# nannau/DoWnGAN

Hardware: AMD Instinct MI355X
Metric: train-step samples/sec (G+D+GP) (higher is better)
Workload: dtype bf16

## Files before the change

downgan_amd/csrc/wgrad.hip:

```cpp
#include "dg_internal.h"

#include <stdlib.h>

struct WGArgs {
  const void* x; const void* u; float* dw;
  long long ldx, ldu;
  int H, W, Ho, Wo, stride, Cin, Cout;
  int u_ps, cps_chunks;
  int Mpix, ppb;
  int nci_t;
  float* db;
  int tri;
  float* dwk[8]; float* dbk[8];
  float* det_ws; const float* det_base; long long det_stride, det_db_off;
  const unsigned char* ex; const unsigned char* eu;
  int grp, ngrp, nunits, gtiles;
};

static void wg_group_order(WGArgs& a, int nco_t, int ntiles, int splits) {
  a.grp = 0;
  if (a.tri || ntiles <= 72) return;
  const int per_co = 3 * a.nci_t;
  int cg = 0;
  for (int c = 1; c <= nco_t; ++c)
    if (nco_t % c == 0 && c * per_co <= 64) cg = c;
  if (!cg) return;
  const double dy_b = (double)a.Mpix * a.Cout, x_b = (double)a.Mpix * a.stride * a.stride * a.Cin;
  const double in_order = 8.0 * dy_b + x_b * (a.nci_t >= 8 ? 1.0 : 8.0 / a.nci_t), grouped = dy_b + x_b * (nco_t / cg);
  if (grouped > 0.8 * in_order) return;
  a.grp = cg * per_co; a.ngrp = nco_t / cg; a.nunits = splits * a.ngrp; a.gtiles = ntiles;
}
static unsigned wg_group_blocks(const WGArgs& a) { return 8u * (unsigned)((a.nunits + 7) / 8) * (unsigned)a.grp; }

__device__ __forceinline__ bool wg_decode(const WGArgs& a, int& bx, int& by) {
  const unsigned lin0 = blockIdx.y * gridDim.x + blockIdx.x;
  if (a.grp) {
    const unsigned xcd = lin0 & 7u, slot = lin0 >> 3;
    const unsigned unit = (slot / (unsigned)a.grp) * 8u + xcd, within = slot % (unsigned)a.grp;
    if (unit >= (unsigned)a.nunits) return false;
    by = (int)(unit / (unsigned)a.ngrp); bx = (int)((unit % (unsigned)a.ngrp) * (unsigned)a.grp + within);
    return true;
  }
  const unsigned lin = gridDim.x <= 72 ? xcd_remap(lin0, gridDim.x * gridDim.y) : lin0;
  bx = (int)(lin % gridDim.x); by = (int)(lin / gridDim.x);
  return true;
}
#define WG_DET_PTR(a, p, by) ((a).det_ws ? (a).det_ws + (long long)(by) * (a).det_stride + ((p) - (a).det_base) : (p))
#define WG_DET_DB(a, by) ((a).det_ws ? (a).det_ws + (long long)(by) * (a).det_stride + (a).det_db_off : (a).db)

typedef __attribute__((address_space(3))) s16x4_t* lds_s16x4_ptr;

typedef __attribute__((ext_vector_type(4))) unsigned int u32x4w_t;
#define WG_OOB_OFF 0x80000000u

template <typename T, int BCO, int BCI, bool ROWSTEP, int KP, bool IM2COL = false>
__global__ __launch_bounds__(256) void wg_kernel(const WGArgs a) {
  constexpr int EPC = DT<T>::EPC;
  constexpr int CPRU = BCO / EPC, CPRX = BCI / EPC;
  constexpr int NU = KP * CPRU / 256, NX = KP * CPRX / 256;
  static_assert(NU >= 1 && NX >= 1, "tile too small");
  constexpr int FA = BCO / 64, FB = BCI / 64;
  constexpr int PADE = sizeof(T) == 2 ? 32 : 0;
  constexpr int LDU = BCO + PADE, LDX = BCI + PADE;
  extern __shared__ __attribute__((aligned(16))) unsigned char wg_dsm[];
  T* const smem = reinterpret_cast<T*>(wg_dsm);

  const int tid = threadIdx.x, lane = tid & 63, wave = tid >> 6;
  const unsigned lin0 = blockIdx.y * gridDim.x + blockIdx.x;
  const unsigned lin = gridDim.x <= 72 ? xcd_remap(lin0, gridDim.x * gridDim.y) : lin0;
  const int bx = (int)(lin % gridDim.x), by = (int)(lin / gridDim.x);
  const int ci_t = IM2COL ? 0 : bx % a.nci_t;
  const int tap = IM2COL ? 4 : (bx / a.nci_t) % 9;
  const int co_t = IM2COL ? bx : bx / (a.nci_t * 9);
  const int co0 = co_t * BCO, ci0 = ci_t * BCI;
  const int dr = tap / 3 - 1, dc = tap % 3 - 1;
  const int pbeg = by * a.ppb;
  const int pend = min(a.Mpix, pbeg + a.ppb);
  const T* __restrict__ X = reinterpret_cast<const T*>(a.x);
  const T* __restrict__ U = reinterpret_cast<const T*>(a.u);

  uint4 ru[NU], rx[NX];
  int s_n = 0, s_ho = 0, s_wo = 0;
  unsigned uoffc[NU], xoffc[NX];
  int xrow[NX];
  constexpr int TPC = EPC / 2;
  unsigned imoff[IM2COL ? NX : 1][TPC];
  if constexpr (ROWSTEP) {
    s_wo = pbeg % a.Wo; const int t = pbeg / a.Wo; s_ho = t % a.Ho; s_n = t / a.Ho;
#pragma unroll
    for (int i = 0; i < NU; ++i) {
      const int e = tid + 256 * i, row = e / CPRU, col = e % CPRU;
      const int co = co0 + col * EPC;
      if (co >= a.Cout) { uoffc[i] = WG_OOB_OFF; continue; }
      if (!a.u_ps) uoffc[i] = (unsigned)(((long long)row * a.ldu + co) * (int)sizeof(T));
      else {
        const int cchunk = co / EPC, q = cchunk / a.cps_chunks, c = cchunk - q * a.cps_chunks;
        uoffc[i] = (unsigned)((((long long)(q >> 1) * (2 * a.Wo) + 2 * row + (q & 1)) * a.ldu + c * EPC) * (int)sizeof(T));
      }
    }
#pragma unroll
    for (int i = 0; i < NX; ++i) {
      const int e = tid + 256 * i, row = e / CPRX, col = e % CPRX;
      const int ci = ci0 + col * EPC;
      xrow[i] = row;
      xoffc[i] = ci < a.Cin ? (unsigned)(((long long)row * a.stride * a.ldx + ci) * (int)sizeof(T)) : WG_OOB_OFF;
      if constexpr (IM2COL) {
#pragma unroll
        for (int tt = 0; tt < TPC; ++tt) {
          const int tp = col * TPC + tt;
          imoff[i][tt] = tp < 9 ? (unsigned)((((long long)(tp / 3) * a.W + row + tp % 3) * a.ldx) * (int)sizeof(T)) : WG_OOB_OFF;
        }
      }
    }
  }
  auto gload_row = [&]() {
    const long long ub = !a.u_ps ? ((long long)(s_n * a.Ho + s_ho) * a.Wo + s_wo) * a.ldu
                                 : ((long long)(s_n * 2 * a.Ho + 2 * s_ho) * (2 * a.Wo) + 2 * s_wo) * a.ldu;
    const int hi = s_ho * a.stride + dr;
    const bool row_ok = (unsigned)hi < (unsigned)a.H;
    const int wi0 = s_wo * a.stride + dc;
    const long long xb = ((long long)(s_n * a.H + hi) * a.W + wi0) * a.ldx;
    __amdgpu_buffer_rsrc_t rU = __builtin_amdgcn_make_buffer_rsrc((void*)(U + ub), 0, (int)WG_OOB_OFF, 0x00020000);
    __amdgpu_buffer_rsrc_t rX = __builtin_amdgcn_make_buffer_rsrc((void*)(X + xb), 0, (int)WG_OOB_OFF, 0x00020000);
#pragma unroll
    for (int i = 0; i < NU; ++i) ru[i] = __builtin_bit_cast(uint4, __builtin_amdgcn_raw_buffer_load_b128(rU, uoffc[i], 0, 0));
    if constexpr (IM2COL) {
      const long long xb2 = ((long long)(s_n * a.H + s_ho - 1) * a.W + s_wo - 1) * a.ldx;
      __amdgpu_buffer_rsrc_t rI = __builtin_amdgcn_make_buffer_rsrc((void*)(X + xb2), 0, (int)WG_OOB_OFF, 0x00020000);
#pragma unroll
      for (int i = 0; i < NX; ++i) {
        const int col = (tid + 256 * i) % CPRX;
        unsigned w[4] = {0u, 0u, 0u, 0u};
#pragma unroll
        for (int tt = 0; tt < TPC; ++tt) {
          const int tp = col * TPC + tt;
          const int hh = s_ho - 1 + tp / 3, ww = s_wo - 1 + xrow[i] + tp % 3;
          const unsigned vo = (tp < 9 && (unsigned)hh < (unsigned)a.H && (unsigned)ww < (unsigned)a.W) ? imoff[i][tt] : WG_OOB_OFF;
          if constexpr (sizeof(T) == 2) {
            unsigned v = __builtin_amdgcn_raw_buffer_load_b32(rI, vo, 0, 0);
            if (tp == 9) v = 0x3f80u;
            w[tt] = v;
          } else {
            typedef __attribute__((ext_vector_type(2))) unsigned int u32x2w_t;
            u32x2w_t v = __builtin_amdgcn_raw_buffer_load_b64(rI, vo, 0, 0);
            if (tp == 9) { v[0] = 0x3f800000u; v[1] = 0u; }
            w[2 * tt] = v[0]; w[2 * tt + 1] = v[1];
          }
        }
        rx[i] = make_uint4(w[0], w[1], w[2], w[3]);
      }
    } else {
#pragma unroll
      for (int i = 0; i < NX; ++i) {
        const int wi = wi0 + xrow[i] * a.stride;
        const unsigned vo = (row_ok && (unsigned)wi < (unsigned)a.W) ? xoffc[i] : WG_OOB_OFF;
// ... 335 lines not shown
    const int hi = s_ho + dr;
    const bool row_ok = (unsigned)hi < (unsigned)a.H;
    const int wi0 = s_wo - 1;
    const long long xb = ((long long)(s_n * a.H + (row_ok ? hi : 0)) * a.W + wi0) * a.ldx;
    __amdgpu_buffer_rsrc_t rU = __builtin_amdgcn_make_buffer_rsrc((void*)(U + ub), 0, (int)WG_OOB_OFF, 0x00020000);
    __amdgpu_buffer_rsrc_t rX = __builtin_amdgcn_make_buffer_rsrc((void*)(X + xb), 0, (int)WG_OOB_OFF, 0x00020000);
#pragma unroll
    for (int i = 0; i < NU; ++i) ru[i] = __builtin_bit_cast(uint4, __builtin_amdgcn_raw_buffer_load_b128(rU, uoffc[i], 0, 0));
#pragma unroll
    for (int i = 0; i < NX; ++i) {
      const int wi = wi0 + xrow[i];
      const unsigned vo = (row_ok && (unsigned)wi < (unsigned)a.W) ? xoffc[i] : WG_OOB_OFF;
      rx[i] = __builtin_bit_cast(uint4, __builtin_amdgcn_raw_buffer_load_b128(rX, vo, 0, 0));
    }
    s_wo += KP;
    if (s_wo >= a.Wo) { s_wo = 0; if (++s_ho == a.Ho) { s_ho = 0; ++s_n; } }
  };
  auto lstore = [&](int buf) {
    T* su = smem + buf * BUF;
    T* sx = su + KP * LDU;
#pragma unroll
    for (int i = 0; i < NU; ++i) {
      const int e = tid + 256 * i, row = e / CPRU, col = e % CPRU;
      if (row < KP) *reinterpret_cast<uint4*>(su + row * LDU + col * EPC) = ru[i];
    }
#pragma unroll
    for (int i = 0; i < NX; ++i) {
      const int e = tid + 256 * i, row = e / CPRX, col = e % CPRX;
      if (row < XR) *reinterpret_cast<uint4*>(sx + row * LDX + col * EPC) = rx[i];
    }
  };

  f32x16_t acc[3][FA][FB];
#pragma unroll
  for (int s = 0; s < 3; ++s)
#pragma unroll
    for (int i = 0; i < FA; ++i)
#pragma unroll
      for (int j = 0; j < FB; ++j)
#pragma unroll
        for (int e = 0; e < 16; ++e) acc[s][i][j][e] = 0.f;

  const int wci = wave;
  const int r32 = lane & 31, h = lane >> 5;
  const int nsteps = (pend - pbeg + KP - 1) / KP;
  if (nsteps <= 0) return;

  gload();
  lstore(0);
  __syncthreads();
  int cur = 0;
  for (int ks = 0; ks < nsteps; ++ks) {
    const bool more = ks + 1 < nsteps;
    if (more) gload();
    const T* su = smem + cur * BUF;
    const T* sx = su + KP * LDU;
    if constexpr (sizeof(T) == 2) {
      const int grp16 = (lane >> 4) & 1, i16 = lane & 15, q = i16 >> 2, pp = i16 & 3;
      typedef __attribute__((ext_vector_type(8))) short s16x8_t;
#pragma unroll
      for (int kk = 0; kk < KP / 16; ++kk) {
        bf16x8_t fa[FA];
        const int k0 = kk * 16 + 8 * h + q;
#pragma unroll
        for (int f = 0; f < FA; ++f) {
          const int ch = 32 * f + 16 * grp16 + 4 * pp;
          s16x4_t lo = __builtin_amdgcn_ds_read_tr16_b64_v4i16((lds_s16x4_ptr)(su + k0 * LDU + ch));
          s16x4_t hi = __builtin_amdgcn_ds_read_tr16_b64_v4i16((lds_s16x4_ptr)(su + (k0 + 4) * LDU + ch));
          s16x8_t v = {lo[0], lo[1], lo[2], lo[3], hi[0], hi[1], hi[2], hi[3]};
          fa[f] = __builtin_bit_cast(bf16x8_t, v);
        }
#pragma unroll
        for (int s = 0; s < 3; ++s) {
          bf16x8_t fb[FB];
#pragma unroll
          for (int f = 0; f < FB; ++f) {
            const int ch = wci * (BCI / 4) + 32 * f + 16 * grp16 + 4 * pp;
            s16x4_t lo = __builtin_amdgcn_ds_read_tr16_b64_v4i16((lds_s16x4_ptr)(sx + (k0 + s) * LDX + ch));
            s16x4_t hi = __builtin_amdgcn_ds_read_tr16_b64_v4i16((lds_s16x4_ptr)(sx + (k0 + s + 4) * LDX + ch));
            s16x8_t v = {lo[0], lo[1], lo[2], lo[3], hi[0], hi[1], hi[2], hi[3]};
            fb[f] = __builtin_bit_cast(bf16x8_t, v);
          }
#pragma unroll
          for (int i = 0; i < FA; ++i)
#pragma unroll
            for (int j = 0; j < FB; ++j)
              acc[s][i][j] = __builtin_amdgcn_mfma_f32_32x32x16_bf16(fa[i], fb[j], acc[s][i][j], 0, 0, 0);
        }
      }
    } else {
#pragma unroll 2
      for (int k = 0; k < KP; k += 2) {
        float fa[FA];
#pragma unroll
        for (int f = 0; f < FA; ++f) fa[f] = su[(k + h) * LDU + 32 * f + r32];
#pragma unroll
        for (int s = 0; s < 3; ++s) {
          float fb[FB];
#pragma unroll
          for (int f = 0; f < FB; ++f) fb[f] = sx[(k + h + s) * LDX + wci * (BCI / 4) + 32 * f + r32];
#pragma unroll
          for (int i = 0; i < FA; ++i)
#pragma unroll
            for (int j = 0; j < FB; ++j)
              acc[s][i][j] = __builtin_amdgcn_mfma_f32_32x32x2f32(fa[i], fb[j], acc[s][i][j], 0, 0, 0);
        }
      }
    }
    if (more) lstore(cur ^ 1);
    __syncthreads();
    cur ^= 1;
  }

  const long long ldw = 9ll * a.Cin;
  float* const dwp = WG_DET_PTR(a, a.dw, by);
#pragma unroll
  for (int s = 0; s < 3; ++s) {
    const int tap = trow * 3 + s;
#pragma unroll
    for (int i = 0; i < FA; ++i)
#pragma unroll
      for (int j = 0; j < FB; ++j) {
        const int ci = ci0 + wci * (BCI / 4) + 32 * j + r32;
#pragma unroll
        for (int reg = 0; reg < 16; ++reg) {
          const int co = co0 + 32 * i + (reg & 3) + 8 * (reg >> 2) + 4 * h;
          if (co < a.Cout && ci < a.Cin) atomicAdd(dwp + (long long)co * ldw + tap * a.Cin + ci, acc[s][i][j][reg]);
        }
      }
  }
}

template <typename T>
static int wg3_launch(WGArgs& a, hipStream_t st) {
  constexpr int BCO = 64, BCI = 128;
  const int nco_t = (a.Cout + BCO - 1) / BCO;
  a.nci_t = (a.Cin + BCI - 1) / BCI;
  const int ntiles = nco_t * 3 * a.nci_t;
  const double flops = 2.0 * 9 * a.Cin * (double)a.Cout * a.Mpix;
  const long long cap = (long long)(flops * 5.4e-4 / (3.0 * BCO * BCI * 4.0));
  int splits = wg_pick_splits(ntiles, 2304, cap, a.Mpix, &a.ppb);
  DetPlan plan; float* lo = nullptr; long long span = 0;
  const int granted = wg_det_begin(a, splits, st, &plan, &lo, &span);
  if (granted < 0) return DG_ERR_LAUNCH;
  if (granted != splits) splits = wg_pick_splits(ntiles, (long long)ntiles * granted, 1ll << 40, a.Mpix, &a.ppb);
  constexpr int PADE = sizeof(T) == 2 ? 32 : 0;
  const int lds = 2 * (32 * (BCO + PADE) + 34 * (BCI + PADE)) * (int)sizeof(T);
  if (lds > 65536) DG_SET_MAX_LDS_ONCE((&wg3_kernel<T, BCO>), lds);
  hipLaunchKernelGGL((wg3_kernel<T, BCO>), dim3(ntiles, splits), dim3(256), lds, st, a);
  if (dg_check_launch() != DG_OK) return DG_ERR_LAUNCH;
  return wg_det_end(a, plan, lo, span, st);
}

template <bool S2>
__global__ __launch_bounds__(256, 2) void wg3w_kernel(const WGArgs a) {
  constexpr int BCO = 128, BCI = 128, KP = 32;
  constexpr int XROWS = S2 ? 65 : KP + 2, NXP = S2 ? 4 : 2, LASTP = 4 * NXP, XALLOC = 4 * (LASTP + 1);
  constexpr int ROWB = 256, SU_B = KP * ROWB, SX_B = XALLOC * ROWB, BUFB = SU_B + SX_B;
  extern __shared__ __attribute__((aligned(16))) unsigned char wgw_dsm[];
  const int tid = threadIdx.x, lane = tid & 63, wave = __builtin_amdgcn_readfirstlane(tid >> 6);
  int bx, by;
  if (!wg_decode(a, bx, by)) return;
  int ci_t = bx % a.nci_t;
  int trow = (bx / a.nci_t) % 3;
  int co_t = bx / (a.nci_t * 3);
  if (a.tri) {
    trow = bx % 3;
    const int p = bx / 3;
    co_t = 0;
    while ((co_t + 1) * (co_t + 2) / 2 <= p) ++co_t;
    ci_t = p - co_t * (co_t + 1) / 2;
  }
  const int co0 = co_t * BCO, ci0 = ci_t * BCI;
  const int dr = trow - 1;
  const int pbeg = by * a.ppb;
  const int pend = min(a.Mpix, pbeg + a.ppb);
  const int nsteps = (pend - pbeg + KP - 1) / KP;
  if (nsteps <= 0) return;
  const char* X = reinterpret_cast<const char*>(a.x);
  const char* U = reinterpret_cast<const char*>(a.u);

  const int drow = lane >> 4, lchunk = (lane & 15) ^ (drow << 2);
  const int lcx = S2 ? (lane & 15) ^ (((((wave & 1) << 1) + (drow >> 1)) & 3) << 2) : lchunk;
  const int lcx_last = S2 ? (lane & 15) ^ ((drow >> 1) << 2) : lchunk;
  unsigned uoff[2], xoff[NXP + 1];
  int xr[NXP + 1];
#pragma unroll
  for (int j = 0; j < 2; ++j) {
    const int row = 4 * (wave + 4 * j) + drow, co = co0 + lchunk * 8;
    if (co >= a.Cout) uoff[j] = WG_OOB_OFF;
    else if (!a.u_ps) uoff[j] = (unsigned)(((long long)row * a.ldu + co) * 2);
    else {
      const int cchunk = co / 8, q = cchunk / a.cps_chunks, c = cchunk - q * a.cps_chunks;
      uoff[j] = (unsigned)((((long long)(q >> 1) * (2 * a.Wo) + 2 * row + (q & 1)) * a.ldu + c * 8) * 2);
    }
  }
#pragma unroll
  for (int j = 0; j <= NXP; ++j) {
    const int row = 4 * (j < NXP ? wave + 4 * j : LASTP) + drow, ci = ci0 + (j < NXP ? lcx : lcx_last) * 8;
    xr[j] = row;
    xoff[j] = (row < XROWS && ci < a.Cin) ? (unsigned)(((long long)row * a.ldx + ci) * 2) : WG_OOB_OFF;
  }
  const unsigned lds0 = (unsigned)__builtin_amdgcn_readfirstlane((int)(unsigned long long)((__attribute__((address_space(3))) unsigned char*)wgw_dsm));
  typedef int i32x4w_t __attribute__((ext_vector_type(4)));
  auto dma = [&](unsigned m0v, unsigned voff, const i32x4w_t& rs) {
    asm volatile("s_mov_b32 m0, %0\n\ts_nop 0\n\tbuffer_load_dwordx4 %1, %2, 0 offen lds" ::"s"(m0v), "v"(voff), "s"(rs) : "memory");
  };
  auto make_rs = [&](const char* base) {
    const unsigned long long b = (unsigned long long)base;
    i32x4w_t rs;
    rs[0] = __builtin_amdgcn_readfirstlane((int)(unsigned)b);
    rs[1] = __builtin_amdgcn_readfirstlane((int)((unsigned)(b >> 32) & 0xffffu));
    rs[2] = (int)WG_OOB_OFF;
    rs[3] = 0x00020000;
    return rs;
  };
  int s_wo = pbeg % a.Wo, s_ho, s_n;
  { const int t = pbeg / a.Wo; s_ho = t % a.Ho; s_n = t / a.Ho; }
  auto issue = [&](int buf, int t) {
    const long long ub = !a.u_ps ? ((long long)(s_n * a.Ho + s_ho) * a.Wo + s_wo) * a.ldu
                                 : ((long long)(s_n * 2 * a.Ho + 2 * s_ho) * (2 * a.Wo) + 2 * s_wo) * a.ldu;
    const int hi = (S2 ? 2 * s_ho : s_ho) + dr;
    const bool row_ok = (unsigned)hi < (unsigned)a.H;
    const int wi0 = (S2 ? 2 * s_wo : s_wo) - 1;
    const long long xb = ((long long)(s_n * a.H + (row_ok ? hi : 0)) * a.W + wi0) * a.ldx;
    const i32x4w_t rsU = make_rs(U + ub * 2), rsX = make_rs(X + xb * 2);
    const unsigned m0b = lds0 + (unsigned)buf * BUFB;
    dma(m0b + (unsigned)wave * 1024u, uoff[0], rsU);
    dma(m0b + (unsigned)(wave + 4) * 1024u, uoff[1], rsU);
#pragma unroll
    for (int j = 0; j < NXP; ++j) {
      const unsigned vo = (row_ok && (unsigned)(wi0 + xr[j]) < (unsigned)a.W) ? xoff[j] : WG_OOB_OFF;
      dma(m0b + SU_B + (unsigned)(wave + 4 * j) * 1024u, vo, rsX);
    }
    if ((t & 3) == wave) {
      const unsigned vo = (row_ok && (unsigned)(wi0 + xr[NXP]) < (unsigned)a.W) ? xoff[NXP] : WG_OOB_OFF;
      dma(m0b + SU_B + (unsigned)LASTP * 1024u, vo, rsX);
    }
    s_wo += KP;
    if (s_wo >= a.Wo) { s_wo = 0; if (++s_ho == a.Ho) { s_ho = 0; ++s_n; } }
  };

  f32x16_t acc[3][4];
#pragma unroll
  for (int s = 0; s < 3; ++s)
#pragma unroll
    for (int f = 0; f < 4; ++f)
#pragma unroll
      for (int e = 0; e < 16; ++e) acc[s][f][e] = 0.f;

  const int h = lane >> 5, grp16 = (lane >> 4) & 1, i16 = lane & 15, q = i16 >> 2, pp = i16 & 3, r32 = lane & 31;
  const int bu = (8 * h + q) * ROWB + (q << 6) + 32 * grp16 + 8 * pp;
  int bxs[3];
#pragma unroll
  for (int s = 0; s < 3; ++s) {
    const int row = S2 ? 2 * (8 * h + q) + s : 8 * h + q + s;
    bxs[s] = SU_B + row * ROWB + ((wave ^ ((S2 ? row >> 1 : row) & 3)) << 6) + 32 * grp16 + 8 * pp;
  }
  constexpr int XK = S2 ? 2 : 1;

  float* const db_out = a.tri ? (a.dbk[co_t] ? WG_DET_PTR(a, a.dbk[co_t], by) : nullptr)
                              : (a.db ? WG_DET_DB(a, by) + co0 : nullptr);
  const bool has_db = db_out != nullptr;
  const int db_group = a.det_ws ? 1 : 3 * (a.tri ? co_t + 1 : a.nci_t);
  const bool db_member = a.det_ws ? (trow == 1 && ci_t == 0) : true;
  int db_cnt = a.det_ws ? 0 : ci_t * 3 + trow;
  float dbacc = 0.f;

  issue(0, 0);
  if (nsteps > 1) issue(1, 1);
  auto wait_older = [&](bool newest_in_flight) {
    if (!newest_in_flight) asm volatile("s_waitcnt vmcnt(0)" ::: "memory");
    else if (S2) asm volatile("s_waitcnt vmcnt(6)" ::: "memory");
    else asm volatile("s_waitcnt vmcnt(4)" ::: "memory");
  };
  wait_older(nsteps > 1);
  __syncthreads();
  int cur = 0;
  typedef __attribute__((ext_vector_type(8))) short s16x8_t;
  for (int ks = 0; ks < nsteps; ++ks) {
    const bool ahead = ks + 2 < nsteps;
    int nb = cur + 2; if (nb >= 3) nb -= 3;
    if (ahead) issue(nb, ks + 2);
    const bool db_now = has_db && db_member && db_cnt == 0;
    db_cnt = db_cnt == 0 ? db_group - 1 : db_cnt - 1;
    const unsigned char* sb = wgw_dsm + cur * BUFB;
    auto read_fb = [&](int s, int kk) {
      const unsigned char* pb = sb + bxs[s] + kk * 16 * XK * ROWB;
      const s16x4_t lo = __builtin_amdgcn_ds_read_tr16_b64_v4i16((lds_s16x4_ptr)(pb));
      const s16x4_t hi = __builtin_amdgcn_ds_read_tr16_b64_v4i16((lds_s16x4_ptr)(pb + 4 * XK * ROWB));
      const s16x8_t v = {lo[0], lo[1], lo[2], lo[3], hi[0], hi[1], hi[2], hi[3]};
      return __builtin_bit_cast(bf16x8_t, v);
    };
    bf16x8_t fb = read_fb(0, 0);
#pragma unroll
    for (int kk = 0; kk < KP / 16; ++kk) {
      bf16x8_t fa[4];
#pragma unroll
      for (int f = 0; f < 4; ++f) {
        const unsigned char* pa = sb + (bu ^ (f << 6)) + kk * 16 * ROWB;
        const s16x4_t lo = __builtin_amdgcn_ds_read_tr16_b64_v4i16((lds_s16x4_ptr)(pa));
        const s16x4_t hi = __builtin_amdgcn_ds_read_tr16_b64_v4i16((lds_s16x4_ptr)(pa + 4 * ROWB));
        const s16x8_t v = {lo[0], lo[1], lo[2], lo[3], hi[0], hi[1], hi[2], hi[3]};
        fa[f] = __builtin_bit_cast(bf16x8_t, v);
      }
      if (db_now) {
#pragma unroll
        for (int f = 0; f < 4; ++f) {
          if (f == wave) {
            const u32x4w_t w4 = __builtin_bit_cast(u32x4w_t, fa[f]);
#pragma unroll
            for (int e = 0; e < 4; ++e) dbacc += __uint_as_float(w4[e] << 16) + __uint_as_float(w4[e] & 0xffff0000u);
          }
        }
      }
#pragma unroll
      for (int s = 0; s < 3; ++s) {
        bf16x8_t fbn = fb;
        const bool last = s == 2 && kk == KP / 16 - 1;
        __builtin_amdgcn_sched_barrier(0);
        if (!last) fbn = read_fb(s == 2 ? 0 : s + 1, s == 2 ? kk + 1 : kk);
        __builtin_amdgcn_sched_barrier(0);
#pragma unroll
        for (int f = 0; f < 4; ++f) acc[s][f] = __builtin_amdgcn_mfma_f32_32x32x16_bf16(fa[f], fb, acc[s][f], 0, 0, 0);
        __builtin_amdgcn_sched_barrier(0);
        fb = fbn;
      }
    }
    wait_older(ahead);
    __syncthreads();
    if (++cur == 3) cur = 0;
  }

  if (has_db && db_member && co0 + 32 * wave + r32 < a.Cout) atomicAdd(db_out + 32 * wave + r32, dbacc);
  const int cin_w = a.tri ? (co_t + 1) * BCI : a.Cin;
  const int cow0 = a.tri ? 0 : co0;
  float* const dw_out = WG_DET_PTR(a, a.tri ? a.dwk[co_t] : a.dw, by);
  const long long ldw = 9ll * cin_w;
  const int ci = ci0 + wave * 32 + r32;
  const unsigned lane_off = (unsigned)((((long long)cow0 + 4 * h) * ldw + ci) * 4);
  const bool ci_ok = ci < cin_w;
#pragma unroll
  for (int s = 0; s < 3; ++s) {
    const int tap = trow * 3 + s;
#pragma unroll
    for (int f = 0; f < 4; ++f)
#pragma unroll
      for (int reg = 0; reg < 16; ++reg) {
        const int cor = 32 * f + (reg & 3) + 8 * (reg >> 2);
        char* const base = reinterpret_cast<char*>(dw_out) + ((long long)cor * ldw + (long long)tap * cin_w) * 4;
        if (ci_ok && co0 + cor + 4 * h < a.Cout) atomicAdd(reinterpret_cast<float*>(base + lane_off), acc[s][f][reg]);
      }
  }
}

template <bool S2>
static int wg3w_launch(WGArgs& a, hipStream_t st) {
  constexpr int BCO = 128, BCI = 128;
  const int nco_t = (a.Cout + BCO - 1) / BCO;
  a.nci_t = (a.Cin + BCI - 1) / BCI;
  const int npairs = a.tri ? nco_t * (nco_t + 1) / 2 : nco_t * a.nci_t;
  const int ntiles = 3 * npairs;
  const double flops = 2.0 * 9 * BCO * (double)BCI * npairs * a.Mpix;
  const long long cap = (long long)(flops * 5.4e-4 / (3.0 * BCO * BCI * 4.0));
  int splits = wg_pick_splits(ntiles, 1536, cap, a.Mpix, &a.ppb);
  DetPlan plan; float* lo = nullptr; long long span = 0;
  const int granted = wg_det_begin(a, splits, st, &plan, &lo, &span);
  if (granted < 0) return DG_ERR_LAUNCH;
  if (granted != splits) splits = wg_pick_splits(ntiles, (long long)ntiles * granted, 1ll << 40, a.Mpix, &a.ppb);
  constexpr int lds = 3 * (32 * 256 + (S2 ? 68 : 36) * 256);
  if (lds > 65536) DG_SET_MAX_LDS_ONCE((&wg3w_kernel<S2>), lds);
  wg_group_order(a, nco_t, ntiles, splits);
  hipLaunchKernelGGL((wg3w_kernel<S2>), a.grp ? dim3(wg_group_blocks(a)) : dim3(ntiles, splits), dim3(256), lds, st, a);
  if (dg_check_launch() != DG_OK) return DG_ERR_LAUNCH;
  return wg_det_end(a, plan, lo, span, st);
}

typedef __attribute__((ext_vector_type(8))) int i32x8w_t;
typedef __attribute__((ext_vector_type(2))) int i32x2w_t;
typedef __attribute__((address_space(3))) i32x2w_t* lds_i32x2_ptr;

template <bool S2>
__global__ __launch_bounds__(256, 2) void wg3w_f8_kernel(const WGArgs a) {
  constexpr int BCO = 128, BCI = 128, KP = 64, ROWB = 128;
  constexpr int XK = S2 ? 2 : 1, XROWS = S2 ? 2 * KP + 1 : KP + 2, NXW = S2 ? 4 : 2, XPIECES = 4 * NXW + 1, XPITCH = S2 ? 1152 : 1024;
  constexpr int SU_B = KP * ROWB, SX_B = XPIECES * XPITCH, BUFB = SU_B + SX_B;
  extern __shared__ __attribute__((aligned(16))) unsigned char wg8_dsm[];
  const int tid = threadIdx.x, lane = tid & 63, wave = __builtin_amdgcn_readfirstlane(tid >> 6);
  int bx, by;
  if (!wg_decode(a, bx, by)) return;
  int ci_t = bx % a.nci_t, trow = (bx / a.nci_t) % 3, co_t = bx / (a.nci_t * 3);
  if (a.tri) {
    trow = bx % 3;
    const int p = bx / 3;
    co_t = 0;
    while ((co_t + 1) * (co_t + 2) / 2 <= p) ++co_t;
    ci_t = p - co_t * (co_t + 1) / 2;
  }
  const int co0 = co_t * BCO, ci0 = ci_t * BCI;
  const int dr = trow - 1;
  const int pbeg = by * a.ppb;
  const int pend = min(a.Mpix, pbeg + a.ppb);
  const int nsteps = (pend - pbeg + KP - 1) / KP;
  if (nsteps <= 0) return;
  const char* X = reinterpret_cast<const char*>(a.x);
  const char* U = reinterpret_cast<const char*>(a.u);

  const int drow = lane >> 3, pchunk = lane & 7;
  const int lchunk = ((((pchunk >> 1) ^ ((drow >> 1) & 3)) << 1) | (pchunk & 1)) * 16;
  const unsigned ulane = (unsigned)(drow * (int)a.ldu + lchunk), xlane = (unsigned)(drow * (int)a.ldx + lchunk);
  const unsigned lds0 = (unsigned)__builtin_amdgcn_readfirstlane((int)(unsigned long long)((__attribute__((address_space(3))) unsigned char*)wg8_dsm));
  typedef int i32x4w_t __attribute__((ext_vector_type(4)));
  auto dma = [&](unsigned m0v, unsigned voff, const i32x4w_t& rs, unsigned soff) {
    asm volatile("s_mov_b32 m0, %0\n\ts_nop 0\n\tbuffer_load_dwordx4 %1, %2, %3 offen lds" ::"s"(m0v), "v"(voff), "s"(rs), "s"(soff) : "memory");
  };
  auto make_rs = [&](const char* base) {
    const unsigned long long b = (unsigned long long)base;
    i32x4w_t rs;
    rs[0] = __builtin_amdgcn_readfirstlane((int)(unsigned)b);
    rs[1] = __builtin_amdgcn_readfirstlane((int)((unsigned)(b >> 32) & 0xffffu));
    rs[2] = (int)WG_OOB_OFF;
    rs[3] = 0x00020000;
    return rs;
  };
  int s_wo = pbeg % a.Wo, s_ho, s_n;
  { const int t = pbeg / a.Wo; s_ho = t % a.Ho; s_n = t / a.Ho; }
  auto issue = [&](int buf, int t) {
    const long long ub = ((long long)(s_n * a.Ho + s_ho) * a.Wo + s_wo) * a.ldu + co0;
    const int hi = XK * s_ho + dr;
    const bool row_ok = (unsigned)hi < (unsigned)a.H;
    const int wi0 = XK * s_wo - 1;
    const long long xb = ((long long)(s_n * a.H + (row_ok ? hi : 0)) * a.W + wi0) * a.ldx + ci0;
    const i32x4w_t rsU = make_rs(U + ub), rsX = make_rs(X + xb);
    const unsigned m0b = lds0 + (unsigned)buf * BUFB;
#pragma unroll
    for (int j = 0; j < 2; ++j) dma(m0b + (unsigned)(wave + 4 * j) * 1024u, ulane, rsU, (unsigned)((wave + 4 * j) * 8 * (int)a.ldu));
#pragma unroll
    for (int j = 0; j < NXW; ++j) {
      const int row0 = 8 * (wave + 4 * j);
      const unsigned vo = (row_ok && (unsigned)(wi0 + row0 + drow) < (unsigned)a.W) ? xlane : WG_OOB_OFF;
      dma(m0b + SU_B + (unsigned)(wave + 4 * j) * (unsigned)XPITCH, vo, rsX, (unsigned)(row0 * (int)a.ldx));
    }
    if ((t & 3) == wave) {
      constexpr int R0 = 8 * (XPIECES - 1);
      const unsigned vo = (row_ok && drow < XROWS - R0 && (unsigned)(wi0 + R0 + drow) < (unsigned)a.W) ? xlane : WG_OOB_OFF;
      dma(m0b + SU_B + (unsigned)(XPIECES - 1) * (unsigned)XPITCH, vo, rsX, (unsigned)(R0 * (int)a.ldx));
    }
    s_wo += KP;
    if (s_wo >= a.Wo) { s_wo = 0; if (++s_ho == a.Ho) { s_ho = 0; ++s_n; } }
  };

  f32x16_t acc[3][4];
#pragma unroll
  for (int s = 0; s < 3; ++s)
#pragma unroll
    for (int f = 0; f < 4; ++f)
#pragma unroll
      for (int e = 0; e < 16; ++e) acc[s][f][e] = 0.f;

  const int h = lane >> 5, G = (lane >> 4) & 1, sl = lane & 15, prow = sl >> 1, low = 16 * G + 8 * (sl & 1), r32 = lane & 31;
  const int bu = (32 * h + prow) * ROWB + (((prow >> 1) & 3) << 5) + low;
  int bxs[3];
#pragma unroll
  for (int s = 0; s < 3; ++s) {
    const int row = XK * (32 * h + prow) + s;
    bxs[s] = SU_B + row * ROWB + (S2 ? (row >> 3) * (XPITCH - 1024) : 0) + ((wave ^ ((row >> 1) & 3)) << 5) + low;
  }
  constexpr int XQ = 8 * XK * ROWB + (S2 ? 2 * (XPITCH - 1024) : 0);
  const unsigned eu4 = *reinterpret_cast<const unsigned*>(a.eu + (co0 >> 5));
  const int sxb = (int)a.ex[(ci0 >> 5) + wave];

  issue(0, 0);
  if (nsteps > 1) issue(1, 1);
  auto wait_older = [&](bool newest_in_flight) {
    if (!newest_in_flight) asm volatile("s_waitcnt vmcnt(0)" ::: "memory");
    else if (S2) asm volatile("s_waitcnt vmcnt(6)" ::: "memory");
    else asm volatile("s_waitcnt vmcnt(4)" ::: "memory");
  };
  wait_older(nsteps > 1);
  __syncthreads();
  int cur = 0;
  for (int ks = 0; ks < nsteps; ++ks) {
    const bool ahead = ks + 2 < nsteps;
    int nb = cur + 2; if (nb >= 3) nb -= 3;
    if (ahead) issue(nb, ks + 2);
    const unsigned char* sb = wg8_dsm + cur * BUFB;
    auto read_frag = [&](int off, int qstep) {
      i32x8w_t v;
#pragma unroll
      for (int q = 0; q < 4; ++q) {
        const i32x2w_t t = __builtin_amdgcn_ds_read_tr8_b64_v2i32((lds_i32x2_ptr)(sb + off + q * qstep));
        v[2 * q] = t[0]; v[2 * q + 1] = t[1];
      }
      return v;
    };
    i32x8w_t fb[3];
#pragma unroll
    for (int s = 0; s < 3; ++s) fb[s] = read_frag(bxs[s], XQ);
#pragma unroll
    for (int f = 0; f < 4; ++f) {
      __builtin_amdgcn_sched_barrier(0);
      const i32x8w_t fa = read_frag(bu ^ (f << 5), 8 * ROWB);
      __builtin_amdgcn_sched_barrier(0);
      const int sua = (int)((eu4 >> (8 * f)) & 0xffu);
#pragma unroll
      for (int s = 0; s < 3; ++s)
        acc[s][f] = __builtin_amdgcn_mfma_scale_f32_32x32x64_f8f6f4(fa, fb[s], acc[s][f], 0, 0, 0, sua, 0, sxb);
      asm volatile("" : "+v"(acc[0][f]), "+v"(acc[1][f]), "+v"(acc[2][f]) :: "memory");
      __builtin_amdgcn_sched_barrier(0);
    }
    wait_older(ahead);
    __syncthreads();
    if (++cur == 3) cur = 0;
  }

  const int cin_w = a.tri ? (co_t + 1) * BCI : a.Cin;
  const int cow0 = a.tri ? 0 : co0;
  float* const dw_out = WG_DET_PTR(a, a.tri ? a.dwk[co_t] : a.dw, by);
  const long long ldw = 9ll * cin_w;
  const int ci = ci0 + wave * 32 + r32;
  const unsigned lane_off = (unsigned)((((long long)cow0 + 4 * h) * ldw + ci) * 4);
#pragma unroll
  for (int s = 0; s < 3; ++s) {
    const int tap = trow * 3 + s;
#pragma unroll
    for (int f = 0; f < 4; ++f)
// ... 145 lines not shown
```

Before: 72.62.

## Add 16x16x32 MFMA variant of weight-grad kernel for strided and dense paths

Adds a SHAPE16 template path to the wide weight-gradient kernel that uses 16x16x32 bf16 MFMAs with an 8x2 accumulator layout and matching LDS swizzles, transposed reads, bias column sums and a permlane32 swap in the epilogue. It is enabled by default for the stride-2 and triangular (dense) cases, while stride-1 stays on 32x32. It also moves the per-row DMA address offsets into a scalar soffset operand, which cuts the per-lane offset registers. The change trades the larger 32x32 MFMA tiles for more, smaller MFMA issues, and adds swizzle and epilogue logic that risks bank conflicts or extra instructions.

```diff
diff --git a/downgan_amd/csrc/wgrad.hip b/downgan_amd/csrc/wgrad.hip
--- a/downgan_amd/csrc/wgrad.hip
+++ b/downgan_amd/csrc/wgrad.hip
@@ -1,6 +1,8 @@
 #include "dg_internal.h"
 
 #include <stdlib.h>
+
+#include <type_traits>
 
 struct WGArgs {
   const void* x; const void* u; float* dw;
@@ -642,7 +644,7 @@
   return wg_det_end(a, plan, lo, span, st);
 }
 
-template <bool S2>
+template <bool S2, bool SHAPE16>
 __global__ __launch_bounds__(256, 2) void wg3w_kernel(const WGArgs a) {
   constexpr int BCO = 128, BCI = 128, KP = 32;
   constexpr int XROWS = S2 ? 65 : KP + 2, NXP = S2 ? 4 : 2, LASTP = 4 * NXP, XALLOC = 4 * (LASTP + 1);
@@ -670,31 +672,28 @@
   const char* X = reinterpret_cast<const char*>(a.x);
   const char* U = reinterpret_cast<const char*>(a.u);
 
-  const int drow = lane >> 4, lchunk = (lane & 15) ^ (drow << 2);
-  const int lcx = S2 ? (lane & 15) ^ (((((wave & 1) << 1) + (drow >> 1)) & 3) << 2) : lchunk;
-  const int lcx_last = S2 ? (lane & 15) ^ ((drow >> 1) << 2) : lchunk;
-  unsigned uoff[2], xoff[NXP + 1];
-  int xr[NXP + 1];
-#pragma unroll
-  for (int j = 0; j < 2; ++j) {
-    const int row = 4 * (wave + 4 * j) + drow, co = co0 + lchunk * 8;
-    if (co >= a.Cout) uoff[j] = WG_OOB_OFF;
-    else if (!a.u_ps) uoff[j] = (unsigned)(((long long)row * a.ldu + co) * 2);
+  const int drow = lane >> 4, lchunk_last = (lane & 15) ^ (drow << 2);
+  const int lchunk = SHAPE16 ? lchunk_last ^ ((wave & 1) << 1) : lchunk_last;
+  const int lcx_last = S2 ? (lane & 15) ^ ((drow >> 1) << 2) : lchunk_last;
+  const int lcx = S2 ? (lane & 15) ^ (((((wave & 1) << 1) + (drow >> 1)) & 3) << 2) ^ (SHAPE16 ? ((wave >> 1) & 1) << 1 : 0) : lchunk;
+  const int urow_mul = a.u_ps ? 2 : 1;
+  unsigned uoff, xoff, xoff_last;
+  {
+    const int co = co0 + lchunk * 8;
+    if (co >= a.Cout) uoff = WG_OOB_OFF;
+    else if (!a.u_ps) uoff = (unsigned)(((long long)drow * a.ldu + co) * 2);
     else {
       const int cchunk = co / 8, q = cchunk / a.cps_chunks, c = cchunk - q * a.cps_chunks;
-      uoff[j] = (unsigned)((((long long)(q >> 1) * (2 * a.Wo) + 2 * row + (q & 1)) * a.ldu + c * 8) * 2);
-    }
-  }
-#pragma unroll
-  for (int j = 0; j <= NXP; ++j) {
-    const int row = 4 * (j < NXP ? wave + 4 * j : LASTP) + drow, ci = ci0 + (j < NXP ? lcx : lcx_last) * 8;
-    xr[j] = row;
-    xoff[j] = (row < XROWS && ci < a.Cin) ? (unsigned)(((long long)row * a.ldx + ci) * 2) : WG_OOB_OFF;
+      uoff = (unsigned)((((long long)(q >> 1) * (2 * a.Wo) + 2 * drow + (q & 1)) * a.ldu + c * 8) * 2);
+    }
+    const int ci = ci0 + lcx * 8, cil = ci0 + lcx_last * 8;
+    xoff = ci < a.Cin ? (unsigned)(((long long)drow * a.ldx + ci) * 2) : WG_OOB_OFF;
+    xoff_last = (4 * LASTP + drow < XROWS && cil < a.Cin) ? (unsigned)(((long long)drow * a.ldx + cil) * 2) : WG_OOB_OFF;
   }
   const unsigned lds0 = (unsigned)__builtin_amdgcn_readfirstlane((int)(unsigned long long)((__attribute__((address_space(3))) unsigned char*)wgw_dsm));
   typedef int i32x4w_t __attribute__((ext_vector_type(4)));
-  auto dma = [&](unsigned m0v, unsigned voff, const i32x4w_t& rs) {
-    asm volatile("s_mov_b32 m0, %0\n\ts_nop 0\n\tbuffer_load_dwordx4 %1, %2, 0 offen lds" ::"s"(m0v), "v"(voff), "s"(rs) : "memory");
+  auto dma = [&](unsigned m0v, unsigned voff, const i32x4w_t& rs, int soff) {
+    asm volatile("s_mov_b32 m0, %0\n\ts_nop 0\n\tbuffer_load_dwordx4 %1, %2, %3 offen lds" ::"s"(m0v), "v"(voff), "s"(rs), "s"(soff) : "memory");
   };
   auto make_rs = [&](const char* base) {
     const unsigned long long b = (unsigned long long)base;
@@ -705,6 +704,7 @@
     rs[3] = 0x00020000;
     return rs;
   };
+  const int urowb = __builtin_amdgcn_readfirstlane(urow_mul * (int)a.ldu * 2), xrowb = __builtin_amdgcn_readfirstlane((int)a.ldx * 2);
   int s_wo = pbeg % a.Wo, s_ho, s_n;
   { const int t = pbeg / a.Wo; s_ho = t % a.Ho; s_n = t / a.Ho; }
   auto issue = [&](int buf, int t) {
@@ -716,36 +716,56 @@
     const long long xb = ((long long)(s_n * a.H + (row_ok ? hi : 0)) * a.W + wi0) * a.ldx;
     const i32x4w_t rsU = make_rs(U + ub * 2), rsX = make_rs(X + xb * 2);
     const unsigned m0b = lds0 + (unsigned)buf * BUFB;
-    dma(m0b + (unsigned)wave * 1024u, uoff[0], rsU);
-    dma(m0b + (unsigned)(wave + 4) * 1024u, uoff[1], rsU);
+#pragma unroll
+    for (int j = 0; j < 2; ++j) {
+      const int row0 = 4 * (wave + 4 * j);
+      dma(m0b + (unsigned)(wave + 4 * j) * 1024u, uoff, rsU, row0 * urowb);
+    }
 #pragma unroll
     for (int j = 0; j < NXP; ++j) {
-      const unsigned vo = (row_ok && (unsigned)(wi0 + xr[j]) < (unsigned)a.W) ? xoff[j] : WG_OOB_OFF;
-      dma(m0b + SU_B + (unsigned)(wave + 4 * j) * 1024u, vo, rsX);
+      const int row0 = 4 * (wave + 4 * j);
+      int col0 = wi0 + row0;
+      asm volatile("" : "+s"(col0));
+      const unsigned vo = (row_ok && (unsigned)(col0 + drow) < (unsigned)a.W) ? xoff : WG_OOB_OFF;
+      dma(m0b + SU_B + (unsigned)(wave + 4 * j) * 1024u, vo, rsX, row0 * xrowb);
     }
     if ((t & 3) == wave) {
-      const unsigned vo = (row_ok && (unsigned)(wi0 + xr[NXP]) < (unsigned)a.W) ? xoff[NXP] : WG_OOB_OFF;
-      dma(m0b + SU_B + (unsigned)LASTP * 1024u, vo, rsX);
+      int col0 = wi0 + 4 * LASTP;
+      asm volatile("" : "+s"(col0));
+      const unsigned vo = (row_ok && (unsigned)(col0 + drow) < (unsigned)a.W) ? xoff_last : WG_OOB_OFF;
+      dma(m0b + SU_B + (unsigned)LASTP * 1024u, vo, rsX, 4 * LASTP * xrowb);
     }
     s_wo += KP;
     if (s_wo >= a.Wo) { s_wo = 0; if (++s_ho == a.Ho) { s_ho = 0; ++s_n; } }
   };
 
-  f32x16_t acc[3][4];
-#pragma unroll
-  for (int s = 0; s < 3; ++s)
-#pragma unroll
-    for (int f = 0; f < 4; ++f)
-#pragma unroll
-      for (int e = 0; e < 16; ++e) acc[s][f][e] = 0.f;
+  typedef __attribute__((ext_vector_type(4))) float f32x4w_t;
+  typename std::conditional<SHAPE16, f32x4w_t[3][8][2], f32x16_t[3][4]>::type acc;
+  if constexpr (SHAPE16) {
+#pragma unroll
+    for (int s = 0; s < 3; ++s)
+#pragma unroll
+      for (int f = 0; f < 8; ++f)
+#pragma unroll
+        for (int n = 0; n < 2; ++n) acc[s][f][n] = f32x4w_t{0.f, 0.f, 0.f, 0.f};
+  } else {
+#pragma unroll
+    for (int s = 0; s < 3; ++s)
+#pragma unroll
+      for (int f = 0; f < 4; ++f)
+#pragma unroll
+        for (int e = 0; e < 16; ++e) acc[s][f][e] = 0.f;
+  }
 
   const int h = lane >> 5, grp16 = (lane >> 4) & 1, i16 = lane & 15, q = i16 >> 2, pp = i16 & 3, r32 = lane & 31;
-  const int bu = (8 * h + q) * ROWB + (q << 6) + 32 * grp16 + 8 * pp;
+  const int pix0 = SHAPE16 ? 4 * grp16 + 16 * h + q : 8 * h + q;
+  const int bu = pix0 * ROWB + (q << 6) + 32 * grp16 + 8 * pp;
   int bxs[3];
 #pragma unroll
   for (int s = 0; s < 3; ++s) {
-    const int row = S2 ? 2 * (8 * h + q) + s : 8 * h + q + s;
-    bxs[s] = SU_B + row * ROWB + ((wave ^ ((S2 ? row >> 1 : row) & 3)) << 6) + 32 * grp16 + 8 * pp;
+    const int row = S2 ? 2 * pix0 + s : pix0 + s;
+    const int krow = S2 ? row >> 1 : row;
+    bxs[s] = SU_B + row * ROWB + ((wave ^ (krow & 3)) << 6) + 32 * (SHAPE16 ? (krow >> 2) & 1 : grp16) + 8 * pp;
   }
   constexpr int XK = S2 ? 2 : 1;
 
@@ -755,7 +775,7 @@
   const int db_group = a.det_ws ? 1 : 3 * (a.tri ? co_t + 1 : a.nci_t);
   const bool db_member = a.det_ws ? (trow == 1 && ci_t == 0) : true;
   int db_cnt = a.det_ws ? 0 : ci_t * 3 + trow;
-  float dbacc = 0.f;
+  float dbacc = 0.f, dbacc1 = 0.f;
 
   issue(0, 0);
   if (nsteps > 1) issue(1, 1);
@@ -775,46 +795,73 @@
     const bool db_now = has_db && db_member && db_cnt == 0;
     db_cnt = db_cnt == 0 ? db_group - 1 : db_cnt - 1;
     const unsigned char* sb = wgw_dsm + cur * BUFB;
-    auto read_fb = [&](int s, int kk) {
-      const unsigned char* pb = sb + bxs[s] + kk * 16 * XK * ROWB;
-      const s16x4_t lo = __builtin_amdgcn_ds_read_tr16_b64_v4i16((lds_s16x4_ptr)(pb));
-      const s16x4_t hi = __builtin_amdgcn_ds_read_tr16_b64_v4i16((lds_s16x4_ptr)(pb + 4 * XK * ROWB));
+    auto read2 = [&](const unsigned char* p, int hi_off) {
+      const s16x4_t lo = __builtin_amdgcn_ds_read_tr16_b64_v4i16((lds_s16x4_ptr)(p));
+      const s16x4_t hi = __builtin_amdgcn_ds_read_tr16_b64_v4i16((lds_s16x4_ptr)(p + hi_off));
       const s16x8_t v = {lo[0], lo[1], lo[2], lo[3], hi[0], hi[1], hi[2], hi[3]};
       return __builtin_bit_cast(bf16x8_t, v);
     };
-    bf16x8_t fb = read_fb(0, 0);
-#pragma unroll
-    for (int kk = 0; kk < KP / 16; ++kk) {
-      bf16x8_t fa[4];
-#pragma unroll
-      for (int f = 0; f < 4; ++f) {
-        const unsigned char* pa = sb + (bu ^ (f << 6)) + kk * 16 * ROWB;
-        const s16x4_t lo = __builtin_amdgcn_ds_read_tr16_b64_v4i16((lds_s16x4_ptr)(pa));
-        const s16x4_t hi = __builtin_amdgcn_ds_read_tr16_b64_v4i16((lds_s16x4_ptr)(pa + 4 * ROWB));
-        const s16x8_t v = {lo[0], lo[1], lo[2], lo[3], hi[0], hi[1], hi[2], hi[3]};
-        fa[f] = __builtin_bit_cast(bf16x8_t, v);
+    auto colsum = [&](const bf16x8_t& frag) {
+      const u32x4w_t w4 = __builtin_bit_cast(u32x4w_t, frag);
+      float t = 0.f;
+#pragma unroll
+      for (int e = 0; e < 4; ++e) t += __uint_as_float(w4[e] << 16) + __uint_as_float(w4[e] & 0xffff0000u);
+      return t;
+    };
+    if constexpr (SHAPE16) {
+      bf16x8_t fb[3][2];
+#pragma unroll
+      for (int n = 0; n < 2; ++n) fb[0][n] = read2(sb + (bxs[0] ^ (n << 5)), 8 * XK * ROWB);
+      bf16x8_t fa = read2(sb + bu, 8 * ROWB);
+#pragma unroll
+      for (int s = 1; s < 3; ++s)
+#pragma unroll
+        for (int n = 0; n < 2; ++n) fb[s][n] = read2(sb + (bxs[s] ^ (n << 5)), 8 * XK * ROWB);
+#pragma unroll
+      for (int f = 0; f < 8; ++f) {
+        bf16x8_t fan = fa;
+        __builtin_amdgcn_sched_barrier(0);
+        if (f < 7) fan = read2(sb + (bu ^ ((f + 1) << 5)), 8 * ROWB);
+        __builtin_amdgcn_sched_barrier(0);
+#pragma unroll
+        for (int s = 0; s < 3; ++s)
+#pragma unroll
+          for (int n = 0; n < 2; ++n) acc[s][f][n] = __builtin_amdgcn_mfma_f32_16x16x32_bf16(fa, fb[s][n], acc[s][f][n], 0, 0, 0);
+        __builtin_amdgcn_sched_barrier(0);
+        fa = fan;
       }
       if (db_now) {
 #pragma unroll
-        for (int f = 0; f < 4; ++f) {
-          if (f == wave) {
-            const u32x4w_t w4 = __builtin_bit_cast(u32x4w_t, fa[f]);
-#pragma unroll
-            for (int e = 0; e < 4; ++e) dbacc += __uint_as_float(w4[e] << 16) + __uint_as_float(w4[e] & 0xffff0000u);
-          }
-        }
-      }
-#pragma unroll
-      for (int s = 0; s < 3; ++s) {
-        bf16x8_t fbn = fb;
-        const bool last = s == 2 && kk == KP / 16 - 1;
-        __builtin_amdgcn_sched_barrier(0);
-        if (!last) fbn = read_fb(s == 2 ? 0 : s + 1, s == 2 ? kk + 1 : kk);
-        __builtin_amdgcn_sched_barrier(0);
-#pragma unroll
-        for (int f = 0; f < 4; ++f) acc[s][f] = __builtin_amdgcn_mfma_f32_32x32x16_bf16(fa[f], fb, acc[s][f], 0, 0, 0);
-        __builtin_amdgcn_sched_barrier(0);
-        fb = fbn;
+        for (int j = 0; j < 2; ++j) {
+          const bf16x8_t fd = read2(sb + (bu ^ ((2 * wave + j) << 5)), 8 * ROWB);
+          if (j) dbacc1 += colsum(fd); else dbacc += colsum(fd);
+        }
+      }
+    } else {
+      auto read_fb = [&](int s, int kk) { return read2(sb + bxs[s] + kk * 16 * XK * ROWB, 4 * XK * ROWB); };
+      bf16x8_t fb = read_fb(0, 0);
+#pragma unroll
+      for (int kk = 0; kk < KP / 16; ++kk) {
+        bf16x8_t fa[4];
+#pragma unroll
+        for (int f = 0; f < 4; ++f) fa[f] = read2(sb + (bu ^ (f << 6)) + kk * 16 * ROWB, 4 * ROWB);
+        if (db_now) {
+#pragma unroll
+          for (int f = 0; f < 4; ++f)
+            if (f == wave) dbacc += colsum(fa[f]);
+        }
+#pragma unroll
+        for (int s = 0; s < 3; ++s) {
+          bf16x8_t fbn = fb;
+          const bool last = s == 2 && kk == KP / 16 - 1;
+          __builtin_amdgcn_sched_barrier(0);
+          if (!last) fbn = read_fb(s == 2 ? 0 : s + 1, s == 2 ? kk + 1 : kk);
+          __builtin_amdgcn_sched_barrier(0);
+#pragma unroll
+          for (int f = 0; f < 4; ++f) acc[s][f] = __builtin_amdgcn_mfma_f32_32x32x16_bf16(fa[f], fb, acc[s][f], 0, 0, 0);
+          __builtin_amdgcn_sched_barrier(0);
+          fb = fbn;
+        }
       }
     }
     wait_older(ahead);
@@ -822,26 +869,68 @@
     if (++cur == 3) cur = 0;
   }
 
-  if (has_db && db_member && co0 + 32 * wave + r32 < a.Cout) atomicAdd(db_out + 32 * wave + r32, dbacc);
+  if constexpr (SHAPE16) {
+    dbacc += __shfl_xor(dbacc, 16); dbacc += __shfl_xor(dbacc, 32);
+    dbacc1 += __shfl_xor(dbacc1, 16); dbacc1 += __shfl_xor(dbacc1, 32);
+    if (has_db && db_member && lane < 32 && co0 + 32 * wave + r32 < a.Cout) atomicAdd(db_out + 32 * wave + r32, grp16 ? dbacc1 : dbacc);
+  } else {
+    if (has_db && db_member && co0 + 32 * wave + r32 < a.Cout) atomicAdd(db_out + 32 * wave + r32, dbacc);
+  }
   const int cin_w = a.tri ? (co_t + 1) * BCI : a.Cin;
   const int cow0 = a.tri ? 0 : co0;
   float* const dw_out = WG_DET_PTR(a, a.tri ? a.dwk[co_t] : a.dw, by);
   const long long ldw = 9ll * cin_w;
   const int ci = ci0 + wave * 32 + r32;
-  const unsigned lane_off = (unsigned)((((long long)cow0 + 4 * h) * ldw + ci) * 4);
   const bool ci_ok = ci < cin_w;
-#pragma unroll
-  for (int s = 0; s < 3; ++s) {
-    const int tap = trow * 3 + s;
-#pragma unroll
-    for (int f = 0; f < 4; ++f)
-#pragma unroll
-      for (int reg = 0; reg < 16; ++reg) {
-        const int cor = 32 * f + (reg & 3) + 8 * (reg >> 2);
-        char* const base = reinterpret_cast<char*>(dw_out) + ((long long)cor * ldw + (long long)tap * cin_w) * 4;
-        if (ci_ok && co0 + cor + 4 * h < a.Cout) atomicAdd(reinterpret_cast<float*>(base + lane_off), acc[s][f][reg]);
-      }
-  }
+  if constexpr (SHAPE16) {
+    const int ci2 = ci0 + wave * 32 + 16 * h + i16;
+    const unsigned lane_off = (unsigned)((((long long)cow0 + 4 * grp16) * ldw + ci2) * 4);
+    const bool ci2_ok = ci2 < cin_w;
+#pragma unroll
+    for (int s = 0; s < 3; ++s) {
+      const int tap = trow * 3 + s;
+#pragma unroll
+      for (int f = 0; f < 8; ++f)
+#pragma unroll
+        for (int reg = 0; reg < 4; ++reg) {
+          const auto sw = __builtin_amdgcn_permlane32_swap(__float_as_uint(acc[s][f][0][reg]), __float_as_uint(acc[s][f][1][reg]), false, false);
+#pragma unroll
+          for (int u = 0; u < 2; ++u) {
+            const int cor = 16 * f + 8 * u + reg;
+            char* const base = reinterpret_cast<char*>(dw_out) + ((long long)cor * ldw + (long long)tap * cin_w) * 4;
+            if (ci2_ok && co0 + cor + 4 * grp16 < a.Cout) atomicAdd(reinterpret_cast<float*>(base + lane_off), __uint_as_float(sw[u]));
+          }
+        }
+    }
+  } else {
+    const unsigned lane_off = (unsigned)((((long long)cow0 + 4 * h) * ldw + ci) * 4);
+#pragma unroll
+    for (int s = 0; s < 3; ++s) {
+      const int tap = trow * 3 + s;
+#pragma unroll
+      for (int f = 0; f < 4; ++f)
+#pragma unroll
+        for (int reg = 0; reg < 16; ++reg) {
+          const int cor = 32 * f + (reg & 3) + 8 * (reg >> 2);
+          char* const base = reinterpret_cast<char*>(dw_out) + ((long long)cor * ldw + (long long)tap * cin_w) * 4;
+          if (ci_ok && co0 + cor + 4 * h < a.Cout) atomicAdd(reinterpret_cast<float*>(base + lane_off), acc[s][f][reg]);
+        }
+    }
+  }
+}
+
+#ifdef DG_WG_SHAPE
+constexpr bool WG3W_S1_16 = DG_WG_SHAPE == 16, WG3W_S2_16 = DG_WG_SHAPE == 16, WG3W_DENSE_16 = DG_WG_SHAPE == 16;
+#else
+constexpr bool WG3W_S1_16 = false, WG3W_S2_16 = true, WG3W_DENSE_16 = true;
+#endif
+
+template <bool S2, bool SHAPE16>
+static int wg3w_go(const WGArgs& a, dim3 grid, hipStream_t st) {
+  constexpr int lds = 3 * (32 * 256 + (S2 ? 68 : 36) * 256);
+  if (lds > 65536) DG_SET_MAX_LDS_ONCE((&wg3w_kernel<S2, SHAPE16>), lds);
+  hipLaunchKernelGGL((wg3w_kernel<S2, SHAPE16>), grid, dim3(256), lds, st, a);
+  return DG_OK;
 }
 
 template <bool S2>
@@ -858,10 +947,13 @@
   const int granted = wg_det_begin(a, splits, st, &plan, &lo, &span);
   if (granted < 0) return DG_ERR_LAUNCH;
   if (granted != splits) splits = wg_pick_splits(ntiles, (long long)ntiles * granted, 1ll << 40, a.Mpix, &a.ppb);
-  constexpr int lds = 3 * (32 * 256 + (S2 ? 68 : 36) * 256);
-  if (lds > 65536) DG_SET_MAX_LDS_ONCE((&wg3w_kernel<S2>), lds);
   wg_group_order(a, nco_t, ntiles, splits);
-  hipLaunchKernelGGL((wg3w_kernel<S2>), a.grp ? dim3(wg_group_blocks(a)) : dim3(ntiles, splits), dim3(256), lds, st, a);
+  const dim3 grid = a.grp ? dim3(wg_group_blocks(a)) : dim3(ntiles, splits);
+  int rc;
+  if constexpr (S2) rc = wg3w_go<true, WG3W_S2_16>(a, grid, st);
+  else if constexpr (WG3W_S1_16 == WG3W_DENSE_16) rc = wg3w_go<false, WG3W_S1_16>(a, grid, st);
+  else rc = a.tri ? wg3w_go<false, WG3W_DENSE_16>(a, grid, st) : wg3w_go<false, WG3W_S1_16>(a, grid, st);
+  if (rc != DG_OK) return rc;
   if (dg_check_launch() != DG_OK) return DG_ERR_LAUNCH;
   return wg_det_end(a, plan, lo, span, st);
 }
```

Result: no change. 73.17, median of 6 (+0.8%).
